# donydchen/matchnerf

Hardware: AMD Instinct MI355X
Metric: rendered rays/sec (3-view, 64 samples/ray) (higher is better)
Workload: dtype f32; 1 GPU

## Files before the change

### include/mnerf.h

```cpp
#ifndef MNERF_H_
#define MNERF_H_

#include <stdint.h>

#ifdef __cplusplus
extern "C" {
#endif

#define MNERF_ABI_VERSION 12
#define MNERF_MAX_VIEWS 16
#define MNERF_FEAT_CH 128
#define MNERF_COND_STRIDE_MAX 96
#define MNERF_COND_STRIDE_MAX_F32 64

enum {
  MNERF_OK = 0,
  MNERF_E_NULL = -1,
  MNERF_E_RANGE = -2,
  MNERF_E_UNSUPPORTED = -3,
  MNERF_E_ALIGN = -4
};

typedef struct mnerf_view {
  float extr[12];
// ... 58 lines not shown

int mnerf_ray_samples(const mnerf_rays* rays, const mnerf_view* view, float* pts, float* ndc,
                      float* depth, void* stream);

int mnerf_composite(int32_t n_rays, int32_t n_samples, const float* rgb_s, const float* sigma,
                    const float* depth_s, const float* ray_len, int32_t wo_render_interval,
                    int32_t setbg_opaque, float* rgb, float* depth, float* opacity, float* prob,
                    void* stream);

int mnerf_cost_volume(const mnerf_scene* scene, const mnerf_rays* rays, int32_t cond_stride,
                      float* cond, void* stream);

int64_t mnerf_cost_volume_operand_bytes(const mnerf_scene* scene);
int mnerf_cost_volume_operands(const mnerf_scene* scene, void* opnd, void* stream);

int64_t mnerf_decoder_wstream_floats(int32_t cond_dim, int32_t cond_stride, int32_t L_3D,
                                     int32_t wstream_format);
int mnerf_decoder_chunk(const mnerf_decoder* dec, const mnerf_view* view0, const mnerf_rays* rays,
                        const float* cond, float* rgb, float* depth, float* opacity,
                        float* dbg_rgb_s, float* dbg_sigma, void* stream);

int mnerf_decoder_samples(const mnerf_decoder* dec, int32_t n_rays, int32_t n_samples,
                          int32_t legacy_coord, const float* x_ndc, const float* dir,
                          const float* cond, float* rgb_s, float* sigma, void* stream);

int64_t mnerf_render_workspace_bytes(int32_t n_rays, int32_t n_samples, int32_t cond_stride);
int32_t mnerf_render_chunk_is_fused(const mnerf_scene* scene, const mnerf_decoder* dec, const mnerf_rays* rays);
int32_t mnerf_render_takes_pose_table(const mnerf_scene* scene, const mnerf_decoder* dec, int32_t n_samples,
                                      int32_t rays_per_pose);
int mnerf_render_chunk(const mnerf_scene* scene, const mnerf_decoder* dec, const mnerf_rays* rays,
                       void* workspace, float* rgb, float* depth, float* opacity, void* stream);
int mnerf_render_chunk_fused(const mnerf_scene* scene, const mnerf_decoder* dec, const mnerf_rays* rays,
                             float* rgb, float* depth, float* opacity, void* stream);

int mnerf_box_downsample(const float* src, int32_t h, int32_t w, int32_t channels, int32_t k, float* dst, void* stream);

#define MNERF_RAY_FLOATS 8
int mnerf_cost_volume_rays(const mnerf_scene* scene, const mnerf_rays* rays, const float* ray_od, int32_t cond_stride, float* cond,
                           void* stream);
int mnerf_ray_samples_rays(const mnerf_rays* rays, const float* ray_od, const mnerf_view* view0, float* x_ndc, float* dir,
                           float* depth_s, float* ray_len, void* stream);
int64_t mnerf_render_rays_workspace_bytes(int32_t n_rays, int32_t n_samples, int32_t cond_stride);
int mnerf_render_rays(const mnerf_scene* scene, const mnerf_decoder* dec, const mnerf_rays* rays, const float* ray_od,
                      void* workspace, float* rgb, float* depth, float* opacity, void* stream);

#define MNERF_CAM_PINHOLE 0
#define MNERF_CAM_FISHEYE 1
#define MNERF_CAM_SPHERE 2
#define MNERF_CAM_ORTHO 3
typedef struct mnerf_camera {
  int32_t model, height, width, legacy_coord;
  float kinv[9];
  float c2w[12];
  float lon_lat[4];
} mnerf_camera;
#define MNERF_STRUCT_CAMERA 32
int mnerf_camera_rays(const void* camera, int32_t pixel_begin, int32_t n_pixels, float* ray_od, void* stream);

int mnerf_composite_backward(int32_t n_rays, int32_t n_samples, const float* rgb_s, const float* sigma,
                             const float* depth_s, const float* ray_len, int32_t wo_render_interval,
                             int32_t setbg_opaque, const float* g_rgb, const float* g_depth,
                             const float* g_opacity, float* g_rgb_s, float* g_sigma, void* stream);
int mnerf_cost_volume_backward(const mnerf_scene* scene, const mnerf_rays* rays, int32_t cond_stride,
                               const float* g_cond, float* g_feat0, float* g_feat1, void* stream);

int mnerf_debug_set_knob(const char* name, int value, int* old_value);
// ... 267 lines not shown
```

### matchnerf_amd/csrc/api.cpp

```cpp
#include <string.h>
#include <stdarg.h>
#include <stdio.h>
#include <stdlib.h>

#include <mutex>

#include "common.hpp"
#include "launch_plan.hpp"

static thread_local char g_err[512] = "";

void mnerf_set_error(const char* fmt, ...) {
  va_list ap;
  va_start(ap, fmt);
  vsnprintf(g_err, sizeof(g_err), fmt, ap);
  va_end(ap);
}

extern "C" int mnerf_abi_version(void) { return MNERF_ABI_VERSION; }
extern "C" const char* mnerf_last_error(void) { return g_err; }

extern "C" int64_t mnerf_struct_size(int32_t which) {
  switch (which) {
    case 0: return (int64_t)sizeof(mnerf_view);
// ... 78 lines not shown
  std::lock_guard<std::mutex> hold(g_tuning_lock);
  return g_tuning;
}

extern "C" int mnerf_debug_set_knob(const char* name, int value, int* old_value) {
  std::lock_guard<std::mutex> hold(g_tuning_lock);
  struct Knob { const char* name; int* slot; };
  const Knob knobs[] = {{"decoder_pp", &g_tuning.decoder_pp}, {"decoder_pp_grid", &g_tuning.decoder_pp_grid},
                        {"decoder_pp_max_s", &g_tuning.decoder_pp_max_s}, {"decoder_grid", &g_tuning.decoder_grid},
                        {"cv_variant", &g_tuning.cv_variant}, {"cv_mm", &g_tuning.cv_mm}, {"cv_mm_spw", &g_tuning.cv_mm_spw}, {"cv_uvpair", &g_tuning.cv_uvpair}, {"cv_pair_block", &g_tuning.cv_pair_block}, {"cv_grid", &g_tuning.cv_grid},
                        {"render_fused", &g_tuning.render_fused}, {"wa_min4", &g_tuning.wa_min4}};
  for (const Knob& k : knobs)
    if (name && strcmp(name, k.name) == 0) {
      if (old_value) *old_value = *k.slot;
      *k.slot = value;
      return MNERF_OK;
    }
  mnerf_set_error("mnerf_debug_set_knob: unknown knob '%s'", name ? name : "(null)");
  return MNERF_E_RANGE;
}

extern "C" int mnerf_debug_launch_plan(const char* what, const int64_t* args, int32_t n_args, int32_t* plan, int32_t n_plan) {
  MNERF_REQUIRE(what && args && plan, MNERF_E_NULL, "mnerf_debug_launch_plan: NULL argument");
  struct Planner { const char* name; int (*fn)(const int64_t*, int32_t, int32_t*, int32_t); };
  const Planner planners[] = {{"conv2d", mnerf_plan_conv2d}, {"conv_gemm", mnerf_plan_conv_gemm}, {"conv_wgrad", mnerf_plan_conv_wgrad},
                              {"instance_norm", mnerf_plan_instance_norm}, {"instance_norm_backward", mnerf_plan_instance_norm},
                              {"window_attention", mnerf_plan_window_attention}};
  for (const Planner& p : planners)
    if (strcmp(what, p.name) == 0) return p.fn(args, n_args, plan, n_plan);
  mnerf_set_error("mnerf_debug_launch_plan: unknown dispatcher '%s'", what);
  return MNERF_E_RANGE;
}

bool mnerf_once_per_device(std::atomic<unsigned long long>& mask) {
  int dev = 0;
  (void)hipGetDevice(&dev);
  const unsigned long long bit = 1ull << (dev & 63);
  return (mask.fetch_or(bit, std::memory_order_relaxed) & bit) == 0;
}
```

### matchnerf_amd/csrc/launch_plan.hpp

```cpp
#pragma once
#include <stdint.h>

int mnerf_plan_conv2d(const int64_t* args, int32_t n_args, int32_t* plan, int32_t n_plan);
int mnerf_plan_conv_gemm(const int64_t* args, int32_t n_args, int32_t* plan, int32_t n_plan);
int mnerf_plan_conv_wgrad(const int64_t* args, int32_t n_args, int32_t* plan, int32_t n_plan);
int mnerf_plan_instance_norm(const int64_t* args, int32_t n_args, int32_t* plan, int32_t n_plan);
int mnerf_plan_window_attention(const int64_t* args, int32_t n_args, int32_t* plan, int32_t n_plan);
```

### matchnerf_amd/csrc/render_chunk.hip

```cpp
#include "common.hpp"

extern "C" int64_t mnerf_render_workspace_bytes(int32_t n_rays, int32_t n_samples,
                                                int32_t cond_stride) {
  if (n_rays < 0 || n_samples < 1 || cond_stride < 1) return -1;
  return (int64_t)n_rays * n_samples * cond_stride * (int64_t)sizeof(float);
}

static int check_render_args(const mnerf_scene* scene, const mnerf_decoder* dec, const mnerf_rays* rays) {
  MNERF_REQUIRE(scene && dec && rays, MNERF_E_NULL, "mnerf_render_chunk: NULL argument struct");
  MNERF_REQUIRE(dec->n_views == scene->n_views, MNERF_E_RANGE,
                "mnerf_render_chunk: decoder packed for %d views, scene has %d", dec->n_views,
                scene->n_views);
  const int sumG = scene->n_group[0] + (scene->n_scales > 1 ? scene->n_group[1] : 0);
  MNERF_REQUIRE(dec->cond_dim == sumG + 4 * scene->n_views, MNERF_E_RANGE,
                "mnerf_render_chunk: cond_dim=%d != sum(cos_n_group)+4V=%d", dec->cond_dim,
                sumG + 4 * scene->n_views);
  return MNERF_OK;
}

extern "C" int32_t mnerf_render_chunk_is_fused(const mnerf_scene* scene, const mnerf_decoder* dec,
                                               const mnerf_rays* rays) {
  if (check_render_args(scene, dec, rays)) return 0;
  return mnerf_fused_render_applies(scene, dec, rays) ? 1 : 0;
}

extern "C" int32_t mnerf_render_takes_pose_table(const mnerf_scene* scene, const mnerf_decoder* dec, int32_t n_samples,
                                                 int32_t rays_per_pose) {
  if (!scene || !dec || n_samples < 1 || rays_per_pose <= 0 || rays_per_pose % 64) return 0;
  if (scene->n_views < 2 || scene->n_views > MNERF_MAX_VIEWS || scene->n_scales < 1 || scene->n_scales > 2) return 0;
  return mnerf_cost_volume_takes_pose_table(scene) && mnerf_decoder_takes_pose_table(dec, n_samples) ? 1 : 0;
}

extern "C" int mnerf_render_chunk_fused(const mnerf_scene* scene, const mnerf_decoder* dec,
                                        const mnerf_rays* rays_in, float* rgb, float* depth,
                                        float* opacity, void* stream) {
  int rc = check_render_args(scene, dec, rays_in);
  if (rc) return rc;
  mnerf_rays canon;
  rc = mnerf_rays_canonical(rays_in, &canon, "mnerf_render_chunk_fused");
  if (rc) return rc;
  const mnerf_rays* rays = &canon;
  MNERF_REQUIRE(rgb && depth && opacity, MNERF_E_NULL, "mnerf_render_chunk_fused: NULL output buffer");
  MNERF_REQUIRE(mnerf_fused_render_applies(scene, dec, rays), MNERF_E_UNSUPPORTED,
                "mnerf_render_chunk_fused: the one-launch form needs the split-fp16 stream, S <= 128, <= 32 conditioning "
                "inputs and cos_n_group entries >= 2 (use mnerf_render_chunk)");
  rc = mnerf_scene_check(scene, rays, "mnerf_render_chunk_fused");
  if (rc) return rc;
  return mnerf_fused_render_launch(scene, dec, rays, rgb, depth, opacity, stream);
}

extern "C" int mnerf_render_chunk(const mnerf_scene* scene, const mnerf_decoder* dec,
                                  const mnerf_rays* rays_in, void* workspace, float* rgb,
                                  float* depth, float* opacity, void* stream) {
  int rc = check_render_args(scene, dec, rays_in);
  if (rc) return rc;
  mnerf_rays canon;
  rc = mnerf_rays_canonical(rays_in, &canon, "mnerf_render_chunk");
  if (rc) return rc;
  const mnerf_rays* rays = &canon;
  MNERF_REQUIRE(rgb && depth && opacity, MNERF_E_NULL, "mnerf_render_chunk: NULL output buffer");
  if (mnerf_tune().render_fused && mnerf_fused_render_applies(scene, dec, rays))
    return mnerf_render_chunk_fused(scene, dec, rays, rgb, depth, opacity, stream);
  MNERF_REQUIRE(workspace, MNERF_E_NULL, "mnerf_render_chunk: workspace is NULL");
// ... 8 lines not shown
```

### matchnerf_amd/hip.py

```python
import contextlib
import ctypes as C
import os

import numpy as np

MNERF_ABI_VERSION = 12
MNERF_POSE_FLOATS = 24
MNERF_RAY_FLOATS = 8
CAM_PINHOLE, CAM_FISHEYE, CAM_SPHERE, CAM_ORTHO = 0, 1, 2, 3
STRUCT_CAMERA = 32
MNERF_OK, MNERF_E_NULL, MNERF_E_RANGE, MNERF_E_UNSUPPORTED, MNERF_E_ALIGN = 0, -1, -2, -3, -4
MNERF_MAX_VIEWS = 16
MNERF_COND_STRIDE_MAX, MNERF_COND_STRIDE_MAX_F32 = 96, 64
SMALL_FIXED = 32

_LIB = None
_LIB_PATH = os.environ.get("MNERF_LIB") or os.path.join(os.path.dirname(os.path.abspath(__file__)), "libmnerf_hip.so")

class MnerfError(RuntimeError):
    pass


class View(C.Structure):
    _fields_ = [("extr", C.c_float * 12), ("intr", C.c_float * 9), ("near_", C.c_float), ("far_", C.c_float)]
# ... 84 lines not shown


class OptimGroup(C.Structure):
    _fields_ = [("lr", C.c_double), ("beta1", C.c_double), ("beta2", C.c_double), ("eps", C.c_double),
                ("weight_decay", C.c_double), ("max_norm", C.c_double), ("n_blocks", C.c_int32), ("pad_", C.c_int32)]



STRUCTS = (View, Rays, Scene, Decoder, EncoderLayer, ConvLayer, DecoderTrain, EncoderLayerTrain, OptimRow, OptimGroup, LpipsWeightTable)
HEADER_STRUCTS = dict(zip(("mnerf_view", "mnerf_rays", "mnerf_scene", "mnerf_decoder", "mnerf_encoder_layer", "mnerf_conv",
                           "mnerf_decoder_train", "mnerf_encoder_layer_train", "mnerf_optim_row", "mnerf_optim_group",
                           "mnerf_lpips_weights"), STRUCTS))

_int, _i32, _i64, _sz, _f32, _vp, _P = C.c_int, C.c_int32, C.c_int64, C.c_size_t, C.c_float, C.c_void_p, C.POINTER
_rows = _vp

SIGNATURES = {
    "mnerf_abi_version": (_int, []),
    "mnerf_last_error": (C.c_char_p, []),
    "mnerf_struct_size": (_i64, [_i32]),
    "mnerf_ray_samples": (_int, [_P(Rays), _P(View)] + [_vp] * 4),
    "mnerf_composite": (_int, [_i32] * 2 + [_vp] * 4 + [_i32] * 2 + [_vp] * 5),
    "mnerf_cost_volume": (_int, [_P(Scene), _P(Rays), _i32, _vp, _vp]),
    "mnerf_cost_volume_operand_bytes": (_i64, [_P(Scene)]),
    "mnerf_cost_volume_operands": (_int, [_P(Scene), _vp, _vp]),
    "mnerf_decoder_wstream_floats": (_i64, [_i32] * 4),
    "mnerf_decoder_chunk": (_int, [_P(Decoder), _P(View), _P(Rays)] + [_vp] * 7),
    "mnerf_decoder_samples": (_int, [_P(Decoder)] + [_i32] * 3 + [_vp] * 6),
    "mnerf_render_workspace_bytes": (_i64, [_i32] * 3),
    "mnerf_render_chunk_is_fused": (_i32, [_P(Scene), _P(Decoder), _P(Rays)]),
    "mnerf_render_takes_pose_table": (_i32, [_P(Scene), _P(Decoder), _i32, _i32]),
    "mnerf_render_chunk": (_int, [_P(Scene), _P(Decoder), _P(Rays)] + [_vp] * 5),
    "mnerf_render_chunk_fused": (_int, [_P(Scene), _P(Decoder), _P(Rays)] + [_vp] * 4),
    "mnerf_box_downsample": (_int, [_vp] + [_i32] * 4 + [_vp] * 2),
    "mnerf_cost_volume_rays": (_int, [_P(Scene), _P(Rays), _vp, _i32, _vp, _vp]),
    "mnerf_ray_samples_rays": (_int, [_P(Rays), _vp, _P(View)] + [_vp] * 5),
    "mnerf_render_rays_workspace_bytes": (_i64, [_i32] * 3),
    "mnerf_render_rays": (_int, [_P(Scene), _P(Decoder), _P(Rays)] + [_vp] * 6),
    "mnerf_camera_rays": (_int, [_vp, _i32, _i32, _vp, _vp]),
    "mnerf_composite_backward": (_int, [_i32] * 2 + [_vp] * 4 + [_i32] * 2 + [_vp] * 6),
    "mnerf_cost_volume_backward": (_int, [_P(Scene), _P(Rays), _i32] + [_vp] * 4),
    "mnerf_debug_set_knob": (_int, [C.c_char_p, _int, _P(_int)]),
    "mnerf_debug_launch_plan": (_int, [C.c_char_p, _vp, _i32, _P(_i32), _i32]),
    "mnerf_decoder_backward_workspace_bytes": (_i64, [_i32] * 2),
    "mnerf_decoder_backward": (_int, [_P(DecoderTrain)] + [_i32] * 2 + [_vp] * 3 + [_i32] + [_vp] * 5),
    "mnerf_window_attention": (_int, [_vp] * 4 + [_i32] * 6 + [_vp]),
    "mnerf_window_attention_workspace_bytes": (_sz, [_i32] * 4),
    "mnerf_window_attention_presplit": (_int, [_vp] * 4 + [_i32] * 5 + [_vp, _sz, _vp]),
    "mnerf_qkv_wstream_floats": (_i64, []),
    "mnerf_qkv_projection": (_int, [_vp, _P(_i32), _vp, _vp, _i32] + [_vp] * 3 + [_i32] * 2 + [_vp]),
    "mnerf_qkv_window_images": (_int, [_vp, _P(_i32), _vp, _vp, _i32, _vp, _vp, _sz] + [_i32] * 5 + [_vp]),
    "mnerf_window_attention_images": (_int, [_vp] * 2 + [_i32] * 5 + [_vp, _sz, _vp]),
    "mnerf_window_attention_backward_workspace_bytes": (_i64, [_i32] * 3),
    "mnerf_window_attention_backward": (_int, [_vp] * 8 + [_i32] * 5 + [_vp, _sz, _vp]),
    "mnerf_window_attention_presplit_stats": (_int, [_vp] * 5 + [_i32] * 5 + [_vp, _sz, _vp]),
    "mnerf_window_attention_backward_stats": (_int, [_vp] * 9 + [_i32] * 5 + [_vp, _sz, _vp]),
    "mnerf_instance_norm": (_int, [_vp] * 3 + [_i64, _i64, _f32, _i32, _i32, _vp, _vp]),
    "mnerf_instance_norm_backward": (_int, [_vp] * 3 + [_i64, _i64, _f32, _i32, _vp]),
    "mnerf_upsample_bilinear2x": (_int, [_vp] * 3 + [_i64, _i32, _i32, _vp]),
    "mnerf_upsample_bilinear2x_backward": (_int, [_vp] * 2 + [_i64, _i32, _i32, _vp]),
    "mnerf_conv_wstream_floats": (_i64, [_i32] * 3),
    "mnerf_conv2d": (_int, [_P(ConvLayer), _vp, _i32, _i32] + [_vp] * 4 + [_i32, _vp] + [_i32] * 3 + [_vp]),
    "mnerf_conv_stem_wstream_floats": (_i64, []),
    "mnerf_conv_stem": (_int, [_vp, _i32] + [_vp] * 3 + [_i32] * 3 + [_vp]),
    "mnerf_absmax": (_int, [_vp, _i64, _vp, _vp]),
    "mnerf_conv2d_backward_data": (_int, [_vp] * 3 + [_i32] * 7 + [_vp]),
# ... 434 lines not shown
    import torch
    lib = load()
    with _on(rgb.device, stream) as st:
        tst = stream if stream is not None else torch.cuda.current_stream(rgb.device)
        if fused:
            if timer is not None:
                e0, e1 = timer.span("render_fused", rays.n_rays)
                e0.record(tst)
            check(lib.mnerf_render_chunk_fused(C.byref(scene), C.byref(dec), C.byref(rays), _ptr(rgb), _ptr(depth),
                                               _ptr(opacity), st), "mnerf_render_chunk_fused")
            if timer is not None:
                e1.record(tst)
            return
        if timer is None:
            check(lib.mnerf_render_chunk(C.byref(scene), C.byref(dec), C.byref(rays), _ptr(workspace), _ptr(rgb),
                                         _ptr(depth), _ptr(opacity), st), "mnerf_render_chunk")
            return
        a0, a1 = timer.span("cost_volume", rays.n_rays)
        a0.record(tst)
        check(lib.mnerf_cost_volume(C.byref(scene), C.byref(rays), dec.cond_stride, _ptr(workspace), st),
              "mnerf_cost_volume")
        a1.record(tst)
        b0, b1 = timer.span("decoder", rays.n_rays)
        b0.record(tst)
        check(lib.mnerf_decoder_chunk(C.byref(dec), C.byref(scene.views[0]), C.byref(rays), _ptr(workspace),
                                      _ptr(rgb), _ptr(depth), _ptr(opacity), None, None, st), "mnerf_decoder_chunk")
        b1.record(tst)


def render_workspace_bytes(n_rays, n_samples, cond_stride):
    return int(load().mnerf_render_workspace_bytes(n_rays, n_samples, cond_stride))




def make_free_rays(n_rays, n_samples, height, width, near, far, legacy=True, depth_inverse=False, strat_u_ptr=None):
    return make_rays(n_rays, n_samples, height, width, np.zeros(9, np.float32), np.zeros(12, np.float32), near, far, legacy=legacy,
                     depth_inverse=depth_inverse, strat_u_ptr=strat_u_ptr)


def _bundle(ray_od, n_rays):
    _f32c(ray_od, "ray_od")
    if ray_od.numel() < n_rays * MNERF_RAY_FLOATS:
        raise MnerfError(f"ray_od {tuple(ray_od.shape)} holds fewer than {n_rays} rows of {MNERF_RAY_FLOATS} floats")
    return ray_od


def camera_rays(cam, pixel_begin=0, n_pixels=None, out=None, device=None, stream=None):
    import torch
    lib = load()
    if n_pixels is None:
        n_pixels = cam.height * cam.width - int(pixel_begin)
    if out is None:
        out = torch.empty(int(n_pixels), MNERF_RAY_FLOATS, device=torch.device(device) if device is not None else _current_device())
    _bundle(out, int(n_pixels))
    with _on(out.device, stream) as st:
        check(lib.mnerf_camera_rays(C.byref(cam), int(pixel_begin), int(n_pixels), _ptr(out), st), "mnerf_camera_rays")
    return out


def cost_volume_rays(scene, rays, ray_od, cond_stride, out=None, stream=None):
    import torch
    lib = load()
    _bundle(ray_od, rays.n_rays)
    if out is None:
        out = torch.empty(rays.n_rays * rays.n_samples, cond_stride, device=ray_od.device)
# ... 1004 lines not shown
```

### matchnerf_amd/matchnerf.py

```python
import os

import numpy as np
import torch

from . import camera, hip
from .cond_nerf import CondNeRF
from .edict import EasyDict as edict
from .gmflow import GMFlow, pair_major_to_view_chunks

MAX_RAYS_PER_LAUNCH = int(os.environ.get("MNERF_MAX_RAYS_PER_LAUNCH", "65536"))
MAX_RAYS_PER_POSE_LAUNCH = int(os.environ.get("MNERF_MAX_RAYS_PER_POSE_LAUNCH", "262144"))
GRAD_RAYS_PER_CALL = 8192


def launch_chunks(batch_size, n_rays, chunk, device, launch):
    out = edict(rgb=torch.empty(batch_size, n_rays, 3, device=device), depth=torch.empty(batch_size, n_rays, 1, device=device),
                opacity=torch.empty(batch_size, n_rays, 1, device=device))
    for b in range(batch_size):
        for c in range(0, n_rays, chunk):
            m = min(chunk, n_rays - c)
            launch(b, c, m, out.rgb[b, c:c + m], out.depth[b, c:c + m], out.opacity[b, c:c + m])
    return out


class SourceSet:

    def __init__(self, key, keyed, n_views, groups):
        self.key, self.keyed, self.n_views = key, keyed, n_views
        ref_images, self.feats = keyed[0], list(keyed[4:])
        self.groups = [groups] if isinstance(groups, int) else list(groups)
        self.host = tuple(MatchNeRF._host(t) for t in keyed[1:4])
        b, v, _, h, w = ref_images.shape
        self.images_cl = torch.zeros(b, v, h, w, 4, device=ref_images.device)
        self.images_cl[..., :3] = ref_images.detach().permute(0, 1, 3, 4, 2)
        self._scenes, self._ops = {}, {}

    def build(self, b, feats_b):
        sc = hip.Scene()
        sc.n_views, sc.n_scales = self.n_views, len(feats_b)
        assert len(self.groups) == len(feats_b), "cos_n_group needs one entry per feature scale"
        for s, f in enumerate(feats_b):
            assert f.is_contiguous()
            sc.fh[s], sc.fw[s] = f.shape[2], f.shape[3]
            sc.n_group[s] = self.groups[s]
            sc.feat[s] = f.data_ptr()
        sc.images = self.images_cl[b].data_ptr()
        ex, it, nf = self.host
        for v in range(self.n_views):
            sc.views[v] = hip.make_view(ex[b, v], it[b, v], nf[b, v, 0], nf[b, v, 1])
        return sc

    def scene(self, b, matrix_form=False):
        if (b, matrix_form) not in self._scenes:
            sc = self._scenes[b, matrix_form] = self.build(b, [f[b] for f in self.feats])
# ... 241 lines not shown

    def render(self, opt, tgt_pose=None, ray_idx=None, mode=None, ref_poses=None, ref_images=None,
               ref_feats_list=None, ray_range=None, tgt_hw=None, ssaa=1):
        if tgt_pose is None:
            raise Exception("Must provide tgt_pose.")
        if not ref_images.is_cuda:
            raise RuntimeError("MatchNeRF.render: the HIP render path needs CUDA tensors (no CPU fallback)")
        batch_size, _, _, img_h, img_w = ref_images.shape
        tgt_h, tgt_w = (img_h, img_w) if tgt_hw is None else (int(tgt_hw[0]), int(tgt_hw[1]))
        device = ref_images.device
        size, ray_kw = self._ray_opts(opt, ref_images)
        n_samples, legacy = size[0], ray_kw["legacy"]
        assert ray_idx is None or ray_range is None
        if int(ssaa) > 1:
            return self._render_ssaa(opt, tgt_pose, int(ssaa), (tgt_h, tgt_w), ray_idx, ray_range, mode, ref_poses, ref_images,
                                     ref_feats_list)
        pix0, n_rays = (0, tgt_h * tgt_w) if ray_range is None else (int(ray_range[0]), int(ray_range[1]))
        if ray_idx is not None:
            n_rays = int(ray_idx.numel())
        idx32 = None if ray_idx is None else ray_idx.to(device=device, dtype=torch.int32).contiguous()
        stratified = mode == "train" and bool(opt.nerf.sample_stratified)

        needs_grad = self._needs_grad(ref_feats_list)
        src = self._sources(ref_poses, ref_images, ref_feats_list)
        tgt_ex, tgt_in, tgt_nf = self._tgt_host(tgt_pose)
        if (needs_grad or mode == "train") and (tgt_h, tgt_w) != (img_h, img_w):
            raise NotImplementedError(f"a target grid {(tgt_h, tgt_w)} other than the views' {(img_h, img_w)} is inference only "
                                      "(the backward kernels answer MNERF_E_UNSUPPORTED)")
        if needs_grad:
            if ray_range is not None:
                ray_idx = torch.arange(pix0, pix0 + n_rays, device=device)
            return self._render_with_grad(opt, src, (tgt_ex, tgt_in, tgt_nf), ray_idx, stratified, ref_images, ref_feats_list, n_rays)
        dec = self._decoder(n_samples, device)
        ws_floats = hip.render_workspace_bytes(min(n_rays, MAX_RAYS_PER_LAUNCH), n_samples, dec.cond_stride) // 4
        consts = [camera.target_ray_consts(tgt_ex[b], tgt_in[b], legacy) for b in range(batch_size)]
        strats = [torch.rand(n_rays, n_samples, device=device) for _ in range(batch_size)] if stratified else None

        def launch(b, c, m, *outs):
            sc = src.scene(b, matrix_form=self.cv_matrix_form and idx32 is None)
            rays = hip.make_rays(m, *size, *consts[b], tgt_nf[b, 0], tgt_nf[b, 1], ray_begin=pix0 + c,
                                 ray_idx_ptr=None if idx32 is None else idx32[c:].data_ptr(),
                                 strat_u_ptr=None if strats is None else strats[b][c:].data_ptr(), tgt_hw=(tgt_h, tgt_w), **ray_kw)
            fused = self.fused_render and hip.render_is_fused(sc, dec, rays)
            hip.render_chunk(sc, dec, rays, None if fused else self._workspace(ws_floats, device), *outs,
                             timer=self.kernel_timer, fused=fused)

        return launch_chunks(batch_size, n_rays, MAX_RAYS_PER_LAUNCH, device, launch)

    def _render_ssaa(self, opt, tgt_pose, k, tgt_hw, ray_idx, ray_range, mode, ref_poses, ref_images, ref_feats_list):
        h, w = tgt_hw
        if ray_idx is not None:
            raise ValueError("render: ssaa > 1 renders full frames or runs of whole rows (ray_range), not a ray_idx list")
        pix0, n = (0, h * w) if ray_range is None else (int(ray_range[0]), int(ray_range[1]))
        if pix0 % w or n % w:
            raise ValueError(f"render: ssaa > 1 needs a ray_range of whole rows, got ({pix0}, {n}) at width {w}")
        hi = self.render(opt, self.resize_pose(tgt_pose, (h, w), (k * h, k * w), bool(opt.nerf.legacy_coord)), mode=mode,
                         ref_poses=ref_poses, ref_images=ref_images, ref_feats_list=ref_feats_list,
                         ray_range=(k * k * pix0, k * k * n), tgt_hw=(k * h, k * w))
        return self._box_filter(hi, n // w, w, k)

    def render_rays(self, opt, ray_o, ray_d, near_far, mode=None, ref_poses=None, ref_images=None, ref_feats_list=None):
        batch_size = ref_images.shape[0]
        self._inference_only(mode, ref_feats_list, "render_rays")
        if not ref_images.is_cuda:
            raise RuntimeError("MatchNeRF.render_rays: the HIP render path needs CUDA tensors (no CPU fallback)")
        device = ref_images.device
        ray_o, ray_d = (torch.as_tensor(t, dtype=torch.float32, device=device) for t in (ray_o, ray_d))
        if ray_o.shape != ray_d.shape or ray_o.shape[-1] != 3 or ray_o.dim() not in (2, 3):
            raise ValueError(f"render_rays: ray_o {tuple(ray_o.shape)} / ray_d {tuple(ray_d.shape)}: both [B,N,3] or [N,3]")
        if ray_o.dim() == 3 and ray_o.shape[0] != batch_size:
            raise ValueError(f"render_rays: {ray_o.shape[0]} ray sets for a batch of {batch_size}")
        if ray_o.dim() == 2:
            shared = camera.ray_bundle(ray_o, ray_d)
            bundles = [shared] * batch_size
        else:
            bundles = [camera.ray_bundle(ray_o[b], ray_d[b]) for b in range(batch_size)]
        nf = np.broadcast_to(self._host(torch.as_tensor(near_far)).reshape(-1, 2), (batch_size, 2))
        return self._render_bundles(opt, bundles, nf, ref_poses, ref_images, ref_feats_list)

    def _inference_only(self, mode, ref_feats_list, who):
# ... 242 lines not shown
```

### matchnerf_amd/csrc/decoder.hip

```cpp
#include "decoder_staged.hpp"

#define PP_STAGES 12
#define PP_PHASES 28
struct PPSched {
  int seg_first[PP_STAGES];
  int n_seg[PP_STAGES];
};

template <int SP>
struct SmemPP {
  static constexpr int TEAM = 128, TILE = 256;
  static constexpr int RING_FLOATS = 4 * SEG_CAP_FLOATS;
  static constexpr int TAIL_F = ((TAIL_FLOATS + 255) / 256) * 256;
  static constexpr int HDR_FLOATS = PP_STAGES * 256;
  static constexpr int RS_FLOATS = TILE * 4;
  static constexpr int TOTAL_FLOATS = RING_FLOATS + TAIL_F + HDR_FLOATS + RS_FLOATS + 64;
  static_assert(TEAM * 64 <= SEG_CAP_FLOATS, "a team's attention scratch must fit one ring slot");
  static_assert(TOTAL_FLOATS * 4 <= 160 * 1024, "LDS budget of one CU");
};
__device__ __host__ constexpr int pp_p0(int s, int fs = 2) {
  if (s == 0) return 1 + 8 * fs;
  constexpr int t[PP_STAGES] = {17, 33, 33, 33, 33, 33, 32, 33, 17, 33, 17, 9};
  return t[s];
}
// ... 243 lines not shown
      const float4 vc = *reinterpret_cast<const float4*>(vb + 4 * g + 4);
#pragma unroll
      for (int u = 0; u < 2; ++u)
#pragma unroll
        for (int r = 0; r < 4; ++r) {
          const float pr = __builtin_amdgcn_exp2f(sc[g + u][r] - m_new);
          sc[g + u][r] = pr;
          ls4[r] += pr;
        }
      oa = mfma4(va.x, sc[g][0], oa);
      ob = mfma4(vc.x, sc[g + 1][0], ob);
      oa = mfma4(va.y, sc[g][1], oa);
      ob = mfma4(vc.y, sc[g + 1][1], ob);
      oa = mfma4(va.z, sc[g][2], oa);
      ob = mfma4(vc.z, sc[g + 1][2], ob);
      oa = mfma4(va.w, sc[g][3], oa);
      ob = mfma4(vc.w, sc[g + 1][3], ob);
    }
    const float f_old = __builtin_amdgcn_exp2f(m_run - m_new);
    const float l_new = l_run * f_old + ((ls4[0] + ls4[1]) + (ls4[2] + ls4[3]));
    f32x4 o_new;
#pragma unroll
    for (int d = 0; d < 4; ++d) o_new[d] = (hsel ? o1[d] : o0[d]) * f_old + (oa[d] + ob[d]);
    if (hsel) {
      m1 = m_new, l1 = l_new, o1 = o_new;
    } else {
      m0 = m_new, l0 = l_new, o0 = o_new;
    }
  }
  {
    const float i0 = 1.0f / l0, i1 = 1.0f / l1;
    *reinterpret_cast<float4*>(o_lds + s_q * 16 + (2 * a_hp) * 4) = make_float4(o0[0] * i0, o0[1] * i0, o0[2] * i0, o0[3] * i0);
    *reinterpret_cast<float4*>(o_lds + s_q * 16 + (2 * a_hp + 1) * 4) = make_float4(o1[0] * i1, o1[1] * i1, o1[2] * i1, o1[3] * i1);
  }
}

template <int SP, int FS = 2, bool POSES = false, int NPK = 3>
__global__ __launch_bounds__(512, 2) void decoder_pp_kernel(
    mnerf_decoder D, DecSched sch, PPSched pps, mnerf_view view0, mnerf_rays Rl, const float* __restrict__ cond,
    float* __restrict__ out_rgb, float* __restrict__ out_depth, float* __restrict__ out_opacity,
    float* __restrict__ dbg_rgb_s, float* __restrict__ dbg_sigma, const float* __restrict__ ext_ndc,
    const float* __restrict__ ext_dir) {
  constexpr int Sp = SP;
  using SM = SmemPP<SP>;
  constexpr int TEAM = SM::TEAM;
  extern __shared__ __attribute__((aligned(16))) float smem[];
  const unsigned ring_lds = __builtin_amdgcn_groupstaticsize();
  const unsigned tail_lds = ring_lds + SM::RING_FLOATS * 4u;
  const unsigned hdr_lds = tail_lds + SM::TAIL_F * 4u;
  float* tail = smem + SM::RING_FLOATS;
  float* rs_all = tail + SM::TAIL_F + SM::HDR_FLOATS;
  float* ln_lds = rs_all + SM::RS_FLOATS;

  const int tid = threadIdx.x;
  const int lane0 = tid & 63;
  const int wave = __builtin_amdgcn_readfirstlane(tid >> 6);
  const int team = wave >> 2, tw = wave & 3;
  const mnerf_rays& R = Rl;
  const int S = R.n_samples;
  constexpr bool WIDE = SP == 256;
  static_assert(!WIDE || (!POSES && FS == 2), "the 256-sample instance exists for the shipped shape without a pose table");
  const int rays_per_team = WIDE ? 0 : TEAM / Sp, rays_per_tile = WIDE ? 1 : 2 * rays_per_team;
  const int n_tiles = (R.n_rays + rays_per_tile - 1) / rays_per_tile;
  const int CS = D.cond_stride;
  const float freq_mul = R.legacy_coord ? 1.0f : 3.14159265358979323846f;
  const float wm1 = (float)(R.width - 1), hm1 = (float)(R.height - 1);
// ... 6 lines not shown
  const float* k_other = smem + (team == 0 ? 2 : 3) * SEG_CAP_FLOATS;
  const float* vt_other = k_other + TEAM * 16;
  float* rows_lds = smem + 1 * SEG_CAP_FLOATS + team * 4096;
  const unsigned rows_lds_addr = ring_lds + (unsigned)(1 * SEG_CAP_FLOATS + team * 4096) * 4u;

#define PP_SLOT_LDS(s_, i_) (ring_lds + (unsigned)(2 * ((s_)&1) + (i_)) * (SEG_CAP_FLOATS * 4u))
#define PP_HDR_LDS(s_) (hdr_lds + (unsigned)(s_) * 1024u)
#define PP_SEG_SRC(s_, i_) (D.wstream + pp_seg_off_floats(s_, i_, FS))

  if (tid < SMALL_FIXED) ln_lds[tid] = D.small_[tid];
  if (tid < 2) reinterpret_cast<unsigned*>(ln_lds)[48 + tid] = 0u;
  const unsigned team_ctr_lds = hdr_lds + (unsigned)(SM::HDR_FLOATS + SM::RS_FLOATS + 48 + team) * 4u;
  int team_epoch = 0;
  const unsigned other_ctr_lds = hdr_lds + (unsigned)(SM::HDR_FLOATS + SM::RS_FLOATS + 48 + (1 - team)) * 4u;
  int tile_it = 0;
  auto wait_other_team = [&](int arrivals) {
    const int want = 4 * arrivals;
    for (;;) {
      unsigned v;
      asm volatile("ds_read_b32 %0, %1\n\ts_waitcnt lgkmcnt(0)" : "=v"(v) : "v"(other_ctr_lds) : "memory");
      if ((int)((unsigned)__builtin_amdgcn_readfirstlane((int)v) - (unsigned)want) >= 0) break;
      __builtin_amdgcn_s_sleep(1);
    }
  };
  {
    const unsigned voff = (unsigned)lane0 * 16u;
    for (int p = wave; p < pp_stream_pieces(19); p += 8)
      glds16_s(D.wstream + pp_stream_off_floats(19, FS) + p * 256, voff, __builtin_amdgcn_readfirstlane(tail_lds + (unsigned)p * 1024u));
    for (int s = wave; s < PP_STAGES; s += 8) glds16_s(PP_SEG_SRC(s, 0), voff, __builtin_amdgcn_readfirstlane(PP_HDR_LDS(s)));
    for (int p = wave; p < pp_p0(0, FS); p += 8)
      glds16_s(PP_SEG_SRC(0, 0) + p * 256, voff, __builtin_amdgcn_readfirstlane(PP_SLOT_LDS(0, 0) + (unsigned)p * 1024u));
  }
  segment_wait();
  __syncthreads();
  if (team == 1) __syncthreads();

  int tile_begin = blockIdx.x, tile_end = n_tiles, tile_step = gridDim.x;
  if (gridDim.x >= 8) {
    const int xcd = blockIdx.x & 7;
    tile_begin = (int)((long long)n_tiles * xcd / 8) + (int)(blockIdx.x >> 3);
    tile_end = (int)((long long)n_tiles * (xcd + 1) / 8);
    tile_step = ((int)gridDim.x - xcd + 7) >> 3;
  }
#ifdef MNERF_TIMELINE
  int pp_tl_tile = -1, pp_ph = 0;
#define PP_STAMPED(sync_)                                                                                      \
  do {                                                                                                         \
    unsigned long long* o_ = (sch.tl && lane0 == 0 && blockIdx.x < 32 && pp_tl_tile >= 0 && pp_tl_tile < 4)     \
                                 ? sch.tl + ((((size_t)blockIdx.x * 4 + pp_tl_tile) * 8 + wave) * PP_PHASES + pp_ph) * 2 \
                                 : nullptr;                                                                    \
    __builtin_amdgcn_sched_barrier(0);                                                                         \
    if (o_) o_[0] = __builtin_amdgcn_s_memtime();                                                              \
    sync_;                                                                                                     \
    if (o_) o_[1] = __builtin_amdgcn_s_memtime();                                                              \
    __builtin_amdgcn_sched_barrier(0);                                                                         \
    ++pp_ph;                                                                                                   \
  } while (0)
#else
#define PP_STAMPED(sync_)                    \
  do {                                       \
    __builtin_amdgcn_sched_barrier(0);       \
    sync_;                                   \
    __builtin_amdgcn_sched_barrier(0);       \
  } while (0)
#endif
#define PP_SYNC() PP_STAMPED(__syncthreads())
// ... 376 lines not shown
      if (hl == 0) {
        const float cr = 1.0f / (1.0f + expf(-c3[0][0] * cc));
        const float cg = 1.0f / (1.0f + expf(-c3[0][1] * cc));
        const float cb = 1.0f / (1.0f + expf(-c3[0][2] * cc));
        rs_lds[s_local * 4 + 0] = cr;
        rs_lds[s_local * 4 + 1] = cg;
        rs_lds[s_local * 4 + 2] = cb;
        if (dbg_rgb_s && ray_ok && jp < S) {
          dbg_rgb_s[gs * 3 + 0] = cr;
          dbg_rgb_s[gs * 3 + 1] = cg;
          dbg_rgb_s[gs * 3 + 2] = cb;
        }
      }
    }
    if (team == 1) {
      segment_wait();
      PP_TSYNC();
    } else {
      PP_SYNC();
    }
    bool next_rows = false;
    if (FS == 2 && S == Sp && has_next) {
      const int first_ray = (tile + tile_step) * rays_per_tile + team * rays_per_team;
      next_rows = WIDE ? first_ray < R.n_rays : first_ray + rays_per_team <= R.n_rays;
      if (next_rows) {
        const float* src = cond + ((size_t)first_ray * S + (WIDE ? team * TEAM : 0)) * CS;
        const int pieces = (TEAM * CS) >> 8;
        for (int p = tw; p < pieces; p += 4) glds16_s_stream(src + p * 256, voff, __builtin_amdgcn_readfirstlane(rows_lds_addr + (unsigned)p * 1024u));
      }
    }
    f32x16 qkv[2];
    qkv[0] = (f32x16)(0.0f);
    qkv[1] = (f32x16)(0.0f);
#pragma unroll
    for (int r = 0; r < 8; ++r) step2(qkv, tail + TAIL_QKV, r, lane, av[r]);
    const float qs = q_valid ? 0.5f * 1.4426950408889634f : 0.0f;
#pragma unroll
    for (int hh = 0; hh < 2; ++hh) {
      const int head = hl + 2 * hh;
      constexpr int SPT = WIDE ? TEAM : SP;
      const int jt = WIDE ? s_local : jp;
      *reinterpret_cast<float4*>(k_lds + ((ray_t * 4 + head) * SPT + jt) * 4) =
          make_float4(qkv[0][8 + 4 * hh], qkv[0][9 + 4 * hh], qkv[0][10 + 4 * hh], qkv[0][11 + 4 * hh]);
      float* vcol = vt_lds + (ray_t * 4 + head) * 4 * SPT + jt;
      vcol[0] = qkv[1][4 * hh];
      vcol[SPT] = qkv[1][4 * hh + 1];
      vcol[2 * SPT] = qkv[1][4 * hh + 2];
      vcol[3 * SPT] = qkv[1][4 * hh + 3];
      *reinterpret_cast<float4*>(q_lds + s_local * 16 + head * 4) =
          make_float4(qkv[0][4 * hh] * qs, qkv[0][4 * hh + 1] * qs, qkv[0][4 * hh + 2] * qs, qkv[0][4 * hh + 3] * qs);
    }
    PP_TSYNC();
    {
      int a_ray, a_hp, a_jq;
      if constexpr (SP >= 64) {
        constexpr int CH = (WIDE ? TEAM : SP) / 64;
        int idx = tw;
        const int chunk = idx % CH;
        idx /= CH;
        a_hp = idx & 1;
        a_ray = idx >> 1;
        a_jq = chunk * 64 + lane;
      } else {
        a_ray = tw;
        a_hp = lane >> 5;
        a_jq = lane & 31;
      }
      if constexpr (WIDE) {
        const float* k0 = team == 0 ? k_lds : k_other;
        const float* vt0 = team == 0 ? vt_lds : vt_other;
        const float* k1 = team == 0 ? k_other : k_lds;
        const float* vt1 = team == 0 ? vt_other : vt_lds;
        const int other_t1 = team == 0 ? 4 * tile_it + 2 : 3 * tile_it + 1;
        auto wait = [&]() { wait_other_team(other_t1); };
        if (S == Sp)
          ray_attention_pp256<false>(q_lds, k0, vt0, k1, vt1, o_lds, a_hp, a_jq, lane, S, team, wait);
        else
          ray_attention_pp256<true>(q_lds, k0, vt0, k1, vt1, o_lds, a_hp, a_jq, lane, S, team, wait);
      } else {
        if (S == Sp)
          ray_attention_pp<SP, false>(q_lds, k_lds, vt_lds, o_lds, a_ray, a_hp, a_ray * Sp + a_jq, lane, S);
        else
          ray_attention_pp<SP, true>(q_lds, k_lds, vt_lds, o_lds, a_ray, a_hp, a_ray * Sp + a_jq, lane, S);
      }
    }
    segment_wait();
    PP_TSYNC();
    {
      float ofc[8];
      {
        const float4* src = reinterpret_cast<const float4*>(o_lds + s_local * 16 + 8 * hl);
        const float4 t0 = src[0], t1 = src[1];
        ofc[0] = t0.x; ofc[1] = t0.y; ofc[2] = t0.z; ofc[3] = t0.w;
        ofc[4] = t1.x; ofc[5] = t1.y; ofc[6] = t1.z; ofc[7] = t1.w;
      }
      float yv[8];
      {
        f32x16 t1 = (f32x16)(0.0f);
#pragma unroll
        for (int t = 0; t < 8; ++t) step1(t1, tail + TAIL_FCO, t, lane, ofc[t]);
        float xs = 0.f;
#pragma unroll
        for (int r = 0; r < 8; ++r) {
          yv[r] = t1[r] + av[r];
          xs += yv[r];
        }
        xs = pair_sum(xs);
        const float mean = xs * (1.0f / 16.0f);
        float var = 0.f;
#pragma unroll
        for (int r = 0; r < 8; ++r) {
          const float dlt = yv[r] - mean;
          var += dlt * dlt;
        }
        var = pair_sum(var);
        const float rstd = 1.0f / sqrtf(var * (1.0f / 16.0f) + 1e-6f);
#pragma unroll
        for (int r = 0; r < 8; ++r) {
          const int o = (r & 3) + 8 * (r >> 2) + 4 * hl;
          yv[r] = (yv[r] - mean) * rstd * ln_lds[o] + ln_lds[16 + o];
        }
      }
      float sigma;
      {
        f32x16 t2 = (f32x16)(0.0f);
#pragma unroll
        for (int r = 0; r < 8; ++r) step1(t2, tail + TAIL_OA0, r, lane, yv[r]);
        step1(t2, tail + TAIL_OA0, 8, lane, hl ? 0.0f : 1.0f);
        f32x16 t3 = (f32x16)(0.0f);
#pragma unroll
        for (int r = 0; r < 8; ++r) {
          float t = t2[r];
          t = D.raytrans_elu ? (t > 0.0f ? t : (expf(t) - 1.0f)) : fmaxf(t, 0.0f);
          step1(t3, tail + TAIL_OA2, r, lane, t);
        }
        step1(t3, tail + TAIL_OA2, 8, lane, hl ? 0.0f : 1.0f);
        sigma = fmaxf(t3[0], 0.0f);
      }
      if (D.density_maskfill && n_valid < 1.0f) sigma = 0.0f;
      if (hl == 0) {
        rs_lds[s_local * 4 + 3] = sigma;
        if (dbg_sigma && ray_ok && jp < S) dbg_sigma[gs] = sigma;
      }
    }
    if (team == 1 && has_next) stage_dma(0, 2);
    PP_TSYNC();
    PP_TILE_RAYS(Rt);
    const int t4_rays = WIDE ? ((team == 1 && tw == 0) ? 1 : 0) : rays_per_team;
    const float* rs_ray = WIDE ? rs_all : rs_lds;
    if (WIDE && t4_rays) wait_other_team(3 * tile_it + 3);
    for (int rt = WIDE ? 0 : tw; rt < t4_rays; rt += 4) {
      const int rr = tile * rays_per_tile + team * rays_per_team + rt;
      if (rr >= R.n_rays || !out_rgb) continue;
      float rlen = 1.0f;
      if (!D.wo_render_interval) {
        const RayGeom gg = make_ray(Rt, rr);
        rlen = sqrtf(gg.rx * gg.rx + gg.ry * gg.ry + gg.rz * gg.rz);
      }
      float carry = 0.f, ar = 0.f, ag = 0.f, ab = 0.f, ad = 0.f, ao = 0.f;
      for (int j0 = 0; j0 < S; j0 += 64) {
        const int jj = j0 + lane;
        const bool ok = jj < S;
        float4 c = make_float4(0.f, 0.f, 0.f, 0.f);
        float dd = 0.f;
        if (ok) {
          c = reinterpret_cast<const float4*>(rs_ray)[rt * Sp + jj];
          dd = sample_depth(Rt, rr, jj);
          if (!D.wo_render_interval) {
            const float intv = (jj + 1 < S) ? (sample_depth(Rt, rr, jj + 1) - dd) : 1e10f;
            c.w = c.w * (intv * rlen);
// ... 191 lines not shown
```

Measured before the change: 12.85 million rays/s.

## Plan render chunk sizes aligned to 4-row blocks and decoder tiling

Adds a host-side planner that, in matrix-form inference, picks the per-launch ray count as a multiple of four target rows. It chooses between rounding the nominal chunk down or up using a cost model of cost-volume row blocks plus decoder tile waves. The aim is to keep the matrix-form cost volume on aligned row blocks and to avoid partial decoder waves at chunk boundaries. Chunk sizes can now exceed the nominal maximum, so the workspace is sized from the largest planned chunk.

```diff
diff --git a/include/mnerf.h b/include/mnerf.h
--- a/include/mnerf.h
+++ b/include/mnerf.h
@@ -114,6 +114,11 @@
                        void* workspace, float* rgb, float* depth, float* opacity, void* stream);
 int mnerf_render_chunk_fused(const mnerf_scene* scene, const mnerf_decoder* dec, const mnerf_rays* rays,
                              float* rgb, float* depth, float* opacity, void* stream);
+
+int32_t mnerf_plan_render_chunks(int32_t tgt_height, int32_t tgt_width, int64_t pix_begin, int64_t n_pix, int32_t n_samples,
+                                 int32_t nominal_rays, int32_t matrix_form, int32_t dec_tile_samples, int32_t dec_workgroups,
+                                 int32_t* chunks, int32_t max_chunks);
+int32_t mnerf_render_decoder_tiling(const mnerf_decoder* dec, int32_t n_samples, int32_t* tile_samples, int32_t* workgroups);
 
 int mnerf_box_downsample(const float* src, int32_t h, int32_t w, int32_t channels, int32_t k, float* dst, void* stream);
 
diff --git a/matchnerf_amd/csrc/api.cpp b/matchnerf_amd/csrc/api.cpp
--- a/matchnerf_amd/csrc/api.cpp
+++ b/matchnerf_amd/csrc/api.cpp
@@ -134,6 +134,55 @@
   return MNERF_E_RANGE;
 }
 
+static long long aligned_plan_cost(long long rows, long long r, long long width, long long rays_per_tile, long long workgroups,
+                                   long long* launches) {
+  auto one = [&](long long m) {
+    long long c = (m + 3) / 4;
+    if (rays_per_tile > 0) c += ((m * width + rays_per_tile - 1) / rays_per_tile + workgroups - 1) / workgroups;
+    return c;
+  };
+  const long long full = rows / r, rest = rows % r;
+  *launches = full + (rest ? 1 : 0);
+  return full * one(r) + (rest ? one(rest) : 0);
+}
+
+extern "C" int32_t mnerf_plan_render_chunks(int32_t tgt_height, int32_t tgt_width, int64_t pix_begin, int64_t n_pix, int32_t n_samples,
+                                            int32_t nominal_rays, int32_t matrix_form, int32_t dec_tile_samples, int32_t dec_workgroups,
+                                            int32_t* chunks, int32_t max_chunks) {
+  MNERF_REQUIRE(n_pix >= 0 && n_samples >= 1 && nominal_rays >= 1 && dec_tile_samples >= 0 && dec_workgroups >= 0 && max_chunks >= 0 &&
+                    (chunks || max_chunks == 0),
+                -1, "mnerf_plan_render_chunks: n_pix=%lld S=%d nominal=%d decoder %d/%d, %d slots at %p", (long long)n_pix, n_samples,
+                nominal_rays, dec_tile_samples, dec_workgroups, max_chunks, (void*)chunks);
+  long long step = nominal_rays;
+  if (matrix_form && n_pix > 0) {
+    const long long W = tgt_width;
+    MNERF_REQUIRE(tgt_height >= 1 && W >= 1 && pix_begin >= 0 && pix_begin + n_pix <= (long long)tgt_height * W, -1,
+                  "mnerf_plan_render_chunks: pixels [%lld, %lld + %lld) outside the %dx%d target grid", (long long)pix_begin,
+                  (long long)pix_begin, (long long)n_pix, tgt_height, tgt_width);
+    if (mnerf_tune().cv_mm && W >= 8 && pix_begin % (4 * W) == 0 && n_pix % W == 0 && n_pix > nominal_rays) {
+      const long long rows = n_pix / W, lo = nominal_rays / (4 * W) * 4, hi = lo * W == nominal_rays ? lo : lo + 4;
+      long long rays_per_tile = 0;
+      if (dec_tile_samples > 0 && dec_workgroups > 0) {
+        int padded = 32;
+        while (padded < n_samples && padded < 256) padded *= 2;
+        rays_per_tile = dec_tile_samples / padded > 0 ? dec_tile_samples / padded : 1;
+      }
+      long long r = hi;
+      if (lo >= 4 && lo != hi) {
+        long long n_lo, n_hi;
+        const long long c_lo = aligned_plan_cost(rows, lo, W, rays_per_tile, dec_workgroups, &n_lo);
+        const long long c_hi = aligned_plan_cost(rows, hi, W, rays_per_tile, dec_workgroups, &n_hi);
+        if (c_lo < c_hi || (c_lo == c_hi && n_lo <= n_hi)) r = lo;
+      }
+      step = r * W;
+    }
+  }
+  const long long n = (n_pix + step - 1) / step;
+  MNERF_REQUIRE(n < (1ll << 31) && step < (1ll << 31), -1, "mnerf_plan_render_chunks: %lld launches of %lld rays", n, step);
+  for (long long i = 0; i < n && i < max_chunks; ++i) chunks[i] = (int32_t)(n_pix - i * step < step ? n_pix - i * step : step);
+  return (int32_t)n;
+}
+
 bool mnerf_once_per_device(std::atomic<unsigned long long>& mask) {
   int dev = 0;
   (void)hipGetDevice(&dev);
diff --git a/matchnerf_amd/csrc/render_chunk.hip b/matchnerf_amd/csrc/render_chunk.hip
--- a/matchnerf_amd/csrc/render_chunk.hip
+++ b/matchnerf_amd/csrc/render_chunk.hip
@@ -29,6 +29,15 @@
   if (!scene || !dec || n_samples < 1 || rays_per_pose <= 0 || rays_per_pose % 64) return 0;
   if (scene->n_views < 2 || scene->n_views > MNERF_MAX_VIEWS || scene->n_scales < 1 || scene->n_scales > 2) return 0;
   return mnerf_cost_volume_takes_pose_table(scene) && mnerf_decoder_takes_pose_table(dec, n_samples) ? 1 : 0;
+}
+
+extern "C" int32_t mnerf_render_decoder_tiling(const mnerf_decoder* dec, int32_t n_samples, int32_t* tile_samples, int32_t* workgroups) {
+  if (!tile_samples || !workgroups) return 0;
+  *tile_samples = *workgroups = 0;
+  if (!dec || n_samples < 1 || !mnerf_decoder_takes_pose_table(dec, n_samples)) return 0;
+  *tile_samples = 256;
+  *workgroups = mnerf_tune().decoder_pp_grid > 0 ? mnerf_tune().decoder_pp_grid : 1;
+  return 1;
 }
 
 extern "C" int mnerf_render_chunk_fused(const mnerf_scene* scene, const mnerf_decoder* dec,
diff --git a/matchnerf_amd/hip.py b/matchnerf_amd/hip.py
--- a/matchnerf_amd/hip.py
+++ b/matchnerf_amd/hip.py
@@ -140,6 +140,8 @@
     "mnerf_render_takes_pose_table": (_i32, [_P(Scene), _P(Decoder), _i32, _i32]),
     "mnerf_render_chunk": (_int, [_P(Scene), _P(Decoder), _P(Rays)] + [_vp] * 5),
     "mnerf_render_chunk_fused": (_int, [_P(Scene), _P(Decoder), _P(Rays)] + [_vp] * 4),
+    "mnerf_plan_render_chunks": (_i32, [_i32] * 2 + [_i64] * 2 + [_i32] * 5 + [_P(_i32), _i32]),
+    "mnerf_render_decoder_tiling": (_i32, [_P(Decoder), _i32, _P(_i32), _P(_i32)]),
     "mnerf_box_downsample": (_int, [_vp] + [_i32] * 4 + [_vp] * 2),
     "mnerf_cost_volume_rays": (_int, [_P(Scene), _P(Rays), _vp, _i32, _vp, _vp]),
     "mnerf_ray_samples_rays": (_int, [_P(Rays), _vp, _P(View)] + [_vp] * 5),
@@ -640,6 +642,24 @@
     return int(load().mnerf_render_workspace_bytes(n_rays, n_samples, cond_stride))
 
 
+def render_decoder_tiling(dec, n_samples):
+    tile, wgs = C.c_int32(0), C.c_int32(0)
+    load().mnerf_render_decoder_tiling(C.byref(dec), int(n_samples), C.byref(tile), C.byref(wgs))
+    return tile.value, wgs.value
+
+
+def plan_render_chunks(n_rays, nominal, n_samples=1, tgt_hw=None, pix_begin=0, dec_tiling=(0, 0)):
+    lib = load()
+    h, w = (0, 0) if tgt_hw is None else (int(tgt_hw[0]), int(tgt_hw[1]))
+    args = (h, w, int(pix_begin), int(n_rays), int(n_samples), int(nominal), int(tgt_hw is not None), int(dec_tiling[0]), int(dec_tiling[1]))
+    n = lib.mnerf_plan_render_chunks(*args, None, 0)
+    if n < 0:
+        raise MnerfError(f"mnerf_plan_render_chunks failed: {lib.mnerf_last_error().decode(errors='replace')}")
+    chunks = (C.c_int32 * max(n, 1))()
+    lib.mnerf_plan_render_chunks(*args, chunks, n)
+    return list(chunks[:n])
+
+
 
 
 def make_free_rays(n_rays, n_samples, height, width, near, far, legacy=True, depth_inverse=False, strat_u_ptr=None):
diff --git a/matchnerf_amd/matchnerf.py b/matchnerf_amd/matchnerf.py
--- a/matchnerf_amd/matchnerf.py
+++ b/matchnerf_amd/matchnerf.py
@@ -16,10 +16,13 @@
 def launch_chunks(batch_size, n_rays, chunk, device, launch):
     out = edict(rgb=torch.empty(batch_size, n_rays, 3, device=device), depth=torch.empty(batch_size, n_rays, 1, device=device),
                 opacity=torch.empty(batch_size, n_rays, 1, device=device))
+    counts = hip.plan_render_chunks(n_rays, chunk) if isinstance(chunk, int) else list(chunk)
+    assert sum(counts) == n_rays
     for b in range(batch_size):
-        for c in range(0, n_rays, chunk):
-            m = min(chunk, n_rays - c)
+        c = 0
+        for m in counts:
             launch(b, c, m, out.rgb[b, c:c + m], out.depth[b, c:c + m], out.opacity[b, c:c + m])
+            c += m
     return out
 
 
@@ -327,12 +330,16 @@
                 ray_idx = torch.arange(pix0, pix0 + n_rays, device=device)
             return self._render_with_grad(opt, src, (tgt_ex, tgt_in, tgt_nf), ray_idx, stratified, ref_images, ref_feats_list, n_rays)
         dec = self._decoder(n_samples, device)
-        ws_floats = hip.render_workspace_bytes(min(n_rays, MAX_RAYS_PER_LAUNCH), n_samples, dec.cond_stride) // 4
+        matrix_form = self.cv_matrix_form and idx32 is None
+        aligned = matrix_form and not stratified and mode != "train"
+        chunks = hip.plan_render_chunks(n_rays, MAX_RAYS_PER_LAUNCH, n_samples, (tgt_h, tgt_w) if aligned else None, pix0,
+                                        hip.render_decoder_tiling(dec, n_samples))
+        ws_floats = hip.render_workspace_bytes(max(chunks, default=0), n_samples, dec.cond_stride) // 4
         consts = [camera.target_ray_consts(tgt_ex[b], tgt_in[b], legacy) for b in range(batch_size)]
         strats = [torch.rand(n_rays, n_samples, device=device) for _ in range(batch_size)] if stratified else None
 
         def launch(b, c, m, *outs):
-            sc = src.scene(b, matrix_form=self.cv_matrix_form and idx32 is None)
+            sc = src.scene(b, matrix_form=matrix_form)
             rays = hip.make_rays(m, *size, *consts[b], tgt_nf[b, 0], tgt_nf[b, 1], ray_begin=pix0 + c,
                                  ray_idx_ptr=None if idx32 is None else idx32[c:].data_ptr(),
                                  strat_u_ptr=None if strats is None else strats[b][c:].data_ptr(), tgt_hw=(tgt_h, tgt_w), **ray_kw)
@@ -340,7 +347,7 @@
             hip.render_chunk(sc, dec, rays, None if fused else self._workspace(ws_floats, device), *outs,
                              timer=self.kernel_timer, fused=fused)
 
-        return launch_chunks(batch_size, n_rays, MAX_RAYS_PER_LAUNCH, device, launch)
+        return launch_chunks(batch_size, n_rays, chunks, device, launch)
 
     def _render_ssaa(self, opt, tgt_pose, k, tgt_hw, ray_idx, ray_range, mode, ref_poses, ref_images, ref_feats_list):
         h, w = tgt_hw
```

Measured after the change: 12.70 million rays/s. 1.1% lower.

## Run decoder tail matmuls on split-fp16 MFMA fragments with per-wave exponent scaling

Applied to the files above, without the earlier changes.

Converts the tail weights (QKV, FC-out, two output-head layers) into split hi/lo half-precision fragments in LDS once at kernel start, with per-matrix power-of-two exponents and biases stored alongside. Per-sample activations are likewise scaled and split, then multiplied through a presplit MFMA path, and the results are rescaled back. The aim is to replace f32 step MFMAs with cheaper f16 MFMA throughput while keeping near-f32 accuracy through the hi/lo split. It adds scaling arithmetic, an extra startup pass with barriers, and a risk of precision loss.

```diff
diff --git a/matchnerf_amd/csrc/decoder.hip b/matchnerf_amd/csrc/decoder.hip
--- a/matchnerf_amd/csrc/decoder.hip
+++ b/matchnerf_amd/csrc/decoder.hip
@@ -299,6 +299,63 @@
     const float i0 = 1.0f / l0, i1 = 1.0f / l1;
     *reinterpret_cast<float4*>(o_lds + s_q * 16 + (2 * a_hp) * 4) = make_float4(o0[0] * i0, o0[1] * i0, o0[2] * i0, o0[3] * i0);
     *reinterpret_cast<float4*>(o_lds + s_q * 16 + (2 * a_hp + 1) * 4) = make_float4(o1[0] * i1, o1[1] * i1, o1[2] * i1, o1[3] * i1);
+  }
+}
+
+#define TAILH_QKV 0u
+#define TAILH_FCO (2u * H16_UNIT_BYTES)
+#define TAILH_OA0 (3u * H16_UNIT_BYTES)
+#define TAILH_OA2 (4u * H16_UNIT_BYTES)
+#define TAILH_BIAS0 2560
+#define TAILH_BIAS2 2576
+#define TAILH_EW 2580
+static_assert(5 * H16_UNIT_BYTES == TAILH_BIAS0 * 4 && TAILH_EW + 4 <= ((TAIL_FLOATS + 255) / 256) * 256, "fragments | biases | exponents");
+__device__ __forceinline__ int tail_weight_exponent(float absmax) {
+  if (!(absmax > 0.0f && absmax < __builtin_inff())) return 0;
+  const int e = __builtin_amdgcn_frexp_expf(absmax);
+  return (H16_TARGET_EXP - 1) - (e < -100 ? -100 : (e > 100 ? 100 : e));
+}
+__device__ __forceinline__ int tail_ew(unsigned tail_lds, int i) {
+  return __builtin_amdgcn_readfirstlane((int)((lds_f32_cptr)(size_t)(tail_lds + (unsigned)(TAILH_EW + i) * 4u))[0]);
+}
+__device__ __forceinline__ PartsH tail_operands(const float (&v)[8], int& eg) {
+  float mx = 0.0f;
+#pragma unroll
+  for (int r = 0; r < 8; ++r) mx = fmaxf(mx, fabsf(v[r]));
+  eg = gain_exp(pair_max(mx));
+  return split8h(v, pow2i(eg));
+}
+__device__ __forceinline__ void tail_fragments_in_place(float* tail, int wave, int lane) {
+  float w[8] = {0.f, 0.f, 0.f, 0.f, 0.f, 0.f, 0.f, 0.f};
+  float bias = 0.0f, mx = 0.0f;
+  if (wave < 2) {
+#pragma unroll
+    for (int j = 0; j < 8; ++j) {
+      const float2 a = reinterpret_cast<const float2*>(tail + TAIL_QKV)[j * 64 + lane];
+      w[j] = wave == 0 ? a.x : a.y;
+      mx = fmaxf(mx, fmaxf(fabsf(a.x), fabsf(a.y)));
+    }
+  } else if (wave < 5) {
+    const float* seg = tail + (wave == 2 ? TAIL_FCO : (wave == 3 ? TAIL_OA0 : TAIL_OA2));
+#pragma unroll
+    for (int j = 0; j < 8; ++j) {
+      w[j] = seg[j * 64 + lane];
+      mx = fmaxf(mx, fabsf(w[j]));
+    }
+    if (wave >= 3) bias = seg[8 * 64 + lane];
+  }
+#pragma unroll
+  for (int d = 32; d >= 1; d >>= 1) mx = fmaxf(mx, __shfl_xor(mx, d));
+  const int ew = tail_weight_exponent(mx);
+  const PartsH p = split8h(w, pow2i(ew));
+  __syncthreads();
+  if (wave < 5) {
+    u32x4* dst = reinterpret_cast<u32x4*>(tail) + wave * (H16_UNIT_BYTES / 16) + lane;
+    dst[0] = __builtin_bit_cast(u32x4, p.hi);
+    dst[64] = __builtin_bit_cast(u32x4, p.lo);
+    if (wave == 3 && lane < 16) tail[TAILH_BIAS0 + lane] = bias;
+    if (wave == 4 && lane == 0) tail[TAILH_BIAS2] = bias;
+    if (wave != 1 && lane == 0) tail[TAILH_EW + (wave == 0 ? 0 : wave - 1)] = (float)ew;
   }
 }
 
@@ -371,6 +428,8 @@
       glds16_s(PP_SEG_SRC(0, 0) + p * 256, voff, __builtin_amdgcn_readfirstlane(PP_SLOT_LDS(0, 0) + (unsigned)p * 1024u));
   }
   segment_wait();
+  __syncthreads();
+  tail_fragments_in_place(tail, wave, lane0);
   __syncthreads();
   if (team == 1) __syncthreads();
 
@@ -813,21 +872,26 @@
     f32x16 qkv[2];
     qkv[0] = (f32x16)(0.0f);
     qkv[1] = (f32x16)(0.0f);
-#pragma unroll
-    for (int r = 0; r < 8; ++r) step2(qkv, tail + TAIL_QKV, r, lane, av[r]);
-    const float qs = q_valid ? 0.5f * 1.4426950408889634f : 0.0f;
+    float cqkv;
+    {
+      int eg;
+      const PartsH pa = tail_operands(av, eg);
+      ksteps_presplit<2, 1>(qkv, tail_lds + TAILH_QKV, lane, &pa);
+      cqkv = pow2i(-(tail_ew(tail_lds, 0) + eg));
+    }
+    const float qs = (q_valid ? 0.5f * 1.4426950408889634f : 0.0f) * cqkv;
 #pragma unroll
     for (int hh = 0; hh < 2; ++hh) {
       const int head = hl + 2 * hh;
       constexpr int SPT = WIDE ? TEAM : SP;
       const int jt = WIDE ? s_local : jp;
       *reinterpret_cast<float4*>(k_lds + ((ray_t * 4 + head) * SPT + jt) * 4) =
-          make_float4(qkv[0][8 + 4 * hh], qkv[0][9 + 4 * hh], qkv[0][10 + 4 * hh], qkv[0][11 + 4 * hh]);
+          make_float4(qkv[0][8 + 4 * hh] * cqkv, qkv[0][9 + 4 * hh] * cqkv, qkv[0][10 + 4 * hh] * cqkv, qkv[0][11 + 4 * hh] * cqkv);
       float* vcol = vt_lds + (ray_t * 4 + head) * 4 * SPT + jt;
-      vcol[0] = qkv[1][4 * hh];
-      vcol[SPT] = qkv[1][4 * hh + 1];
-      vcol[2 * SPT] = qkv[1][4 * hh + 2];
-      vcol[3 * SPT] = qkv[1][4 * hh + 3];
+      vcol[0] = qkv[1][4 * hh] * cqkv;
+      vcol[SPT] = qkv[1][4 * hh + 1] * cqkv;
+      vcol[2 * SPT] = qkv[1][4 * hh + 2] * cqkv;
+      vcol[3 * SPT] = qkv[1][4 * hh + 3] * cqkv;
       *reinterpret_cast<float4*>(q_lds + s_local * 16 + head * 4) =
           make_float4(qkv[0][4 * hh] * qs, qkv[0][4 * hh + 1] * qs, qkv[0][4 * hh + 2] * qs, qkv[0][4 * hh + 3] * qs);
     }
@@ -877,13 +941,16 @@
       }
       float yv[8];
       {
-        f32x16 t1 = (f32x16)(0.0f);
-#pragma unroll
-        for (int t = 0; t < 8; ++t) step1(t1, tail + TAIL_FCO, t, lane, ofc[t]);
+        f32x16 t1[1];
+        t1[0] = (f32x16)(0.0f);
+        int eg;
+        const PartsH po = tail_operands(ofc, eg);
+        ksteps_presplit<1, 1>(t1, tail_lds + TAILH_FCO, lane, &po);
+        const float cfc = pow2i(-(tail_ew(tail_lds, 1) + eg));
         float xs = 0.f;
 #pragma unroll
         for (int r = 0; r < 8; ++r) {
-          yv[r] = t1[r] + av[r];
+          yv[r] = t1[0][r] * cfc + av[r];
           xs += yv[r];
         }
         xs = pair_sum(xs);
@@ -904,19 +971,36 @@
       }
       float sigma;
       {
-        f32x16 t2 = (f32x16)(0.0f);
-#pragma unroll
-        for (int r = 0; r < 8; ++r) step1(t2, tail + TAIL_OA0, r, lane, yv[r]);
-        step1(t2, tail + TAIL_OA0, 8, lane, hl ? 0.0f : 1.0f);
-        f32x16 t3 = (f32x16)(0.0f);
-#pragma unroll
-        for (int r = 0; r < 8; ++r) {
-          float t = t2[r];
-          t = D.raytrans_elu ? (t > 0.0f ? t : (expf(t) - 1.0f)) : fmaxf(t, 0.0f);
-          step1(t3, tail + TAIL_OA2, r, lane, t);
+        f32x16 t2[1];
+        t2[0] = (f32x16)(0.0f);
+        int eg0;
+        {
+          lds_v4f32_cptr bp = (lds_v4f32_cptr)(size_t)(tail_lds + TAILH_BIAS0 * 4u) + hl;
+          const v4f32 b0 = bp[0], b1 = bp[2];
+          const PartsH py = tail_operands(yv, eg0);
+          eg0 += tail_ew(tail_lds, 2);
+          const float bm = pow2i(eg0);
+          t2[0][0] = b0.x * bm; t2[0][1] = b0.y * bm; t2[0][2] = b0.z * bm; t2[0][3] = b0.w * bm;
+          t2[0][4] = b1.x * bm; t2[0][5] = b1.y * bm; t2[0][6] = b1.z * bm; t2[0][7] = b1.w * bm;
+          ksteps_presplit<1, 1>(t2, tail_lds + TAILH_OA0, lane, &py);
         }
-        step1(t3, tail + TAIL_OA2, 8, lane, hl ? 0.0f : 1.0f);
-        sigma = fmaxf(t3[0], 0.0f);
+        float zv[8];
+        {
+          const float c0 = pow2i(-eg0);
+#pragma unroll
+          for (int r = 0; r < 8; ++r) {
+            const float t = t2[0][r] * c0;
+            zv[r] = D.raytrans_elu ? (t > 0.0f ? t : (expf(t) - 1.0f)) : fmaxf(t, 0.0f);
+          }
+        }
+        f32x16 t3[1];
+        t3[0] = (f32x16)(0.0f);
+        int eg2;
+        const PartsH pz = tail_operands(zv, eg2);
+        eg2 += tail_ew(tail_lds, 3);
+        t3[0][0] = hl ? 0.0f : ((lds_f32_cptr)(size_t)(tail_lds + TAILH_BIAS2 * 4u))[0] * pow2i(eg2);
+        ksteps_presplit<1, 1>(t3, tail_lds + TAILH_OA2, lane, &pz);
+        sigma = fmaxf(t3[0][0] * pow2i(-eg2), 0.0f);
       }
       if (D.density_maskfill && n_valid < 1.0f) sigma = 0.0f;
       if (hl == 0) {
```

New measurement: 13.28 million rays/s before, 13.45 million rays/s after (median of 6 runs). 1.3% higher.
